# OpenGVLab/MM-Interleaved

Hardware: NVIDIA H100
Metric: interleaved_steps_per_sec (higher is better)
Workload: dtype bf16

## Files before the change

### mm-interleaved_b200/csrc/attn_fwd_sm100.cu

```cuda
#include "attn_common.cuh"

namespace mmfs {

constexpr int kBM = 128, kBN = 64;
constexpr int kAttnThreads = 288;
constexpr int kConsumers = 256;

template <int HD> constexpr int attn_ctas_per_sm() { return HD == 64 ? 2 : 1; }

template <typename T, int HD>
__global__ void __launch_bounds__(kAttnThreads, attn_ctas_per_sm<HD>())
attn_fwd_kernel(const __grid_constant__ CUtensorMap map_q, const __grid_constant__ CUtensorMap map_k,
                const __grid_constant__ CUtensorMap map_v, const AttnParams p, unsigned *__restrict__ sched, int n_work) {
    constexpr int NBOX = HD / 64;
    constexpr uint32_t QBOX_BYTES = kBM * 128, KBOX_BYTES = kBN * 128;
    constexpr uint32_t Q_BYTES = NBOX * QBOX_BYTES, KV_BYTES = NBOX * KBOX_BYTES;
    extern __shared__ __align__(1024) uint8_t smem_raw[];
    if ((s_addr(smem_raw) & 1023u) != 0u) { asm volatile("trap;"); }
    uint8_t *sQ = smem_raw;
    uint8_t *sK = sQ + Q_BYTES;
    uint8_t *sV = sK + 2 * KV_BYTES;
    uint64_t *bars = reinterpret_cast<uint64_t *>(sV + 2 * KV_BYTES);
    uint64_t *q_full = bars + 0, *q_empty = bars + 1, *k_full = bars + 2 , *k_empty = bars + 4 ,
             *v_full = bars + 6 , *v_empty = bars + 8 , *item_full = bars + 10 , *item_empty = bars + 12 ;
    int *s_item = reinterpret_cast<int *>(bars + 14);

    const int warp = threadIdx.x >> 5, lane = threadIdx.x & 31;
    const int n_q = (p.Tq + kBM - 1) / kBM;
    auto decode = [&](int w, int &h, int &b, int &q0, int &n_tiles) {
        b = w / (n_q * p.H);
        const int r = w - b * (n_q * p.H);
        const int mi = r / p.H;
        h = r - mi * p.H;
        q0 = (p.causal ? n_q - 1 - mi : mi) * kBM;
        int kv_end = p.Tkv;
        if (p.causal) kv_end = min(p.Tkv, p.past + min(q0 + kBM, p.Tq));
        n_tiles = (kv_end + kBN - 1) / kBN;
    };

    if (threadIdx.x == 0) {
        bar_init(q_full, 1);
        bar_init(q_empty, kConsumers);
        for (int i = 0; i < 2; ++i) {
            bar_init(k_full + i, 1); bar_init(v_full + i, 1); bar_init(k_empty + i, kConsumers); bar_init(v_empty + i, kConsumers);
            bar_init(item_full + i, 1); bar_init(item_empty + i, kConsumers);
        }
        asm volatile("fence.mbarrier_init.release.cluster;" ::: "memory");
    }
    __syncthreads();

    if (warp == 8) {
        if (lane == 0) {
            int w = blockIdx.x;
            int g = 0;
            for (int qn = 0;; ++qn) {
                const int slot = qn & 1;
                if (qn >= 2) bar_wait(item_empty + slot, ((qn >> 1) - 1) & 1);
                s_item[slot] = w < n_work ? w : -1;
                bar_arrive(item_full + slot);
                if (w >= n_work) break;
                const int w_next = sched ? (int)gridDim.x + (int)atomicAdd(sched, 1u) : n_work;
                int h, b, q0, n_tiles;
                decode(w, h, b, q0, n_tiles);
                if (qn > 0) bar_wait(q_empty, (qn - 1) & 1);
                bar_expect_tx(q_full, Q_BYTES);
#pragma unroll
                for (int bx = 0; bx < NBOX; ++bx) tma_load_4d(sQ + bx * QBOX_BYTES, &map_q, q_full, bx * 64, h, q0, b);
                for (int j = 0; j < n_tiles; ++j, ++g) {
                    const int s = g & 1;
                    const uint32_t ph = (g >> 1) & 1;
                    bar_wait(k_empty + s, ph ^ 1);
                    bar_expect_tx(k_full + s, KV_BYTES);
#pragma unroll
                    for (int bx = 0; bx < NBOX; ++bx)
                        tma_load_4d(sK + s * KV_BYTES + bx * KBOX_BYTES, &map_k, k_full + s, bx * 64, h, j * kBN, b);
                    bar_wait(v_empty + s, ph ^ 1);
                    bar_expect_tx(v_full + s, KV_BYTES);
#pragma unroll
                    for (int bx = 0; bx < NBOX; ++bx)
                        tma_load_4d(sV + s * KV_BYTES + bx * KBOX_BYTES, &map_v, v_full + s, bx * 64, h, j * kBN, b);
                }
                w = w_next;
            }
        }
        return;
    }

    const int wg = warp >> 2;
    const int quad = lane >> 2, tq = lane & 3;
    const int row_in_tile = wg * 64 + (warp & 3) * 16 + quad;
    const uint32_t q_base = s_addr(sQ) + wg * 64 * 128;
    int g = 0;
    for (int qn = 0;; ++qn) {
        const int slot = qn & 1;
        bar_wait(item_full + slot, (qn >> 1) & 1);
        const int w = s_item[slot];
        bar_arrive(item_empty + slot);
        if (w < 0) break;
        int h, b, q0, n_tiles;
        decode(w, h, b, q0, n_tiles);
        const int r0 = q0 + row_in_tile;
        float m_run[2] = {-INFINITY, -INFINITY}, l_run[2] = {0.f, 0.f};
        float o[HD / 2];
#pragma unroll
        for (int i = 0; i < HD / 2; ++i) o[i] = 0.f;
        bar_wait(q_full, qn & 1);
        if (n_tiles == 0) bar_arrive(q_empty);

        for (int j = 0; j < n_tiles; ++j, ++g) {
            const int s = g & 1;
            const int k0 = j * kBN;
            float sc[kBN / 2];
            bar_wait(k_full + s, (g >> 1) & 1);
            wgmma_fence();
#pragma unroll
            for (int kk = 0; kk < HD / 16; ++kk)
                Wgmma<T>::ss_n64(sc, smem_desc(q_base + (kk >> 2) * QBOX_BYTES + (kk & 3) * 32, 16, 1024),
                                 smem_desc(s_addr(sK) + s * KV_BYTES + (kk >> 2) * KBOX_BYTES + (kk & 3) * 32, 16, 1024), kk > 0);
            wgmma_commit();
            wgmma_wait<0>();
            reg_fence(sc);
            bar_arrive(k_empty + s);
            if (j + 1 == n_tiles) bar_arrive(q_empty);

            const bool need_mask = (k0 + kBN > p.Tkv) || (p.key_mask != nullptr) ||
                                   (p.causal && k0 + kBN - 1 > p.past + q0 + wg * 64);
            if (need_mask) {
#pragma unroll
                for (int jj = 0; jj < kBN / 8; ++jj)
#pragma unroll
                    for (int c = 0; c < 2; ++c) {
                        const int key = k0 + jj * 8 + 2 * tq + c;
                        bool vis = key < p.Tkv;
                        if (vis && p.key_mask != nullptr) vis = p.key_mask[(long)b * p.Tkv + key] != 0;
#pragma unroll
                        for (int i = 0; i < 2; ++i) {
                            const bool ok = vis && (!p.causal || key <= p.past + r0 + 8 * i);
                            if (!ok) sc[jj * 4 + 2 * i + c] = -INFINITY;
                        }
                    }
            }
            float alpha[2], neg_m[2];
#pragma unroll
            for (int i = 0; i < 2; ++i) {
                float mx = -INFINITY;
#pragma unroll
                for (int jj = 0; jj < kBN / 8; ++jj) mx = fmaxf(mx, fmaxf(sc[jj * 4 + 2 * i], sc[jj * 4 + 2 * i + 1]));
                mx = fmaxf(mx, __shfl_xor_sync(0xffffffffu, mx, 1));
                mx = fmaxf(mx, __shfl_xor_sync(0xffffffffu, mx, 2));
                const float m_new = fmaxf(m_run[i], mx);
                alpha[i] = (m_new == -INFINITY) ? 1.f : fast_exp2((m_run[i] - m_new) * p.scale_log2e);
                m_run[i] = m_new;
                neg_m[i] = (m_new == -INFINITY) ? 0.f : -m_new * p.scale_log2e;
            }
            uint32_t pa[kBN / 16][4];
            float ls[2] = {0.f, 0.f};
#pragma unroll
            for (int jj = 0; jj < kBN / 8; ++jj)
#pragma unroll
                for (int i = 0; i < 2; ++i) {
                    const float e0 = fast_exp2(fmaf(sc[jj * 4 + 2 * i], p.scale_log2e, neg_m[i]));
                    const float e1 = fast_exp2(fmaf(sc[jj * 4 + 2 * i + 1], p.scale_log2e, neg_m[i]));
                    ls[i] += e0 + e1;
                    pa[jj >> 1][(jj & 1) * 2 + i] = pack2<T>(e0, e1);
                }
#pragma unroll
            for (int i = 0; i < 2; ++i) l_run[i] = l_run[i] * alpha[i] + ls[i];
#pragma unroll
            for (int jj = 0; jj < HD / 8; ++jj) {
                o[jj * 4 + 0] *= alpha[0]; o[jj * 4 + 1] *= alpha[0];
                o[jj * 4 + 2] *= alpha[1]; o[jj * 4 + 3] *= alpha[1];
            }

            bar_wait(v_full + s, (g >> 1) & 1);
            reg_fence(o);
            wgmma_fence();
#pragma unroll
            for (int kk = 0; kk < kBN / 16; ++kk) {
                const uint64_t dv = smem_desc(s_addr(sV) + s * KV_BYTES + kk * 16 * 128, KBOX_BYTES, 1024);
                if constexpr (HD == 64) Wgmma<T>::rs_n64(o, pa[kk], dv, 1);
                else Wgmma<T>::rs_n128(o, pa[kk], dv, 1);
            }
            wgmma_commit();
            wgmma_wait<0>();
            reg_fence(o);
            bar_arrive(v_empty + s);
        }

        T *out = static_cast<T *>(p.out) + (long)b * p.o_bs + (long)h * HD;
#pragma unroll
        for (int i = 0; i < 2; ++i) {
            float l = l_run[i];
            l += __shfl_xor_sync(0xffffffffu, l, 1);
            l += __shfl_xor_sync(0xffffffffu, l, 2);
            const float inv = (l > 0.f) ? 1.f / l : 0.f;
            const int q = r0 + 8 * i;
            if (q < p.Tq) {
                T *op = out + (long)q * p.o_ts + 2 * tq;
#pragma unroll
                for (int jj = 0; jj < HD / 8; ++jj)
                    *reinterpret_cast<uint32_t *>(op + jj * 8) = pack2<T>(o[jj * 4 + 2 * i] * inv, o[jj * 4 + 2 * i + 1] * inv);
            }
        }
    }
}

struct MapKey {
    const void *ptr; int dtype, B, T, H, hd, box_rows; long bs, ts;
    bool operator==(const MapKey &o) const {
        return ptr == o.ptr && dtype == o.dtype && B == o.B && T == o.T && H == o.H && hd == o.hd && box_rows == o.box_rows &&
               bs == o.bs && ts == o.ts;
    }
};
constexpr int kMapCache = 32;
static thread_local MapKey g_map_keys[kMapCache];
static thread_local CUtensorMap g_map_vals[kMapCache];
static thread_local int g_map_n = 0, g_map_next = 0;

static int make_map_uncached(CUtensorMap *map, const void *ptr, int dtype, int B, int T, int H, int hd, long bs, long ts, int box_rows);

static int make_map(CUtensorMap *map, const void *ptr, int dtype, int B, int T, int H, int hd, long bs, long ts, int box_rows) {
    const MapKey key{ptr, dtype, B, T, H, hd, box_rows, bs, ts};
    for (int i = 0; i < g_map_n; ++i)
        if (g_map_keys[i] == key) { *map = g_map_vals[i]; return MMFS_OK; }
    const int rc = make_map_uncached(map, ptr, dtype, B, T, H, hd, bs, ts, box_rows);
    if (rc != MMFS_OK) return rc;
    g_map_keys[g_map_next] = key;
    g_map_vals[g_map_next] = *map;
    g_map_next = (g_map_next + 1) % kMapCache;
    if (g_map_n < kMapCache) ++g_map_n;
    return MMFS_OK;
}

static int make_map_uncached(CUtensorMap *map, const void *ptr, int dtype, int B, int T, int H, int hd, long bs, long ts, int box_rows) {
    EncodeTiledFn fn = tensor_map_encoder();
    if (!fn) { set_error("attn: cuTensorMapEncodeTiled is not available from this driver"); return MMFS_ECUDA; }
    const cuuint64_t dims[4] = {(cuuint64_t)hd, (cuuint64_t)H, (cuuint64_t)T, (cuuint64_t)B};
    const cuuint64_t strides[3] = {(cuuint64_t)hd * 2, (cuuint64_t)ts * 2, (cuuint64_t)bs * 2};
    const cuuint32_t box[4] = {64, 1, (cuuint32_t)box_rows, 1};
    const cuuint32_t estr[4] = {1, 1, 1, 1};
    CUresult r = fn(map, dtype == MMFS_BF16 ? CU_TENSOR_MAP_DATA_TYPE_BFLOAT16 : CU_TENSOR_MAP_DATA_TYPE_FLOAT16, 4,
                    const_cast<void *>(ptr), dims, strides, box, estr, CU_TENSOR_MAP_INTERLEAVE_NONE,
                    CU_TENSOR_MAP_SWIZZLE_128B, CU_TENSOR_MAP_L2_PROMOTION_L2_128B, CU_TENSOR_MAP_FLOAT_OOB_FILL_NONE);
    if (r != CUDA_SUCCESS) { set_error("attn: cuTensorMapEncodeTiled failed (%d)", (int)r); return MMFS_ECUDA; }
    return MMFS_OK;
}

template <typename T, int HD>
static int launch_attn(const CUtensorMap &mq, const CUtensorMap &mk, const CUtensorMap &mv, const AttnParams &p,
                       unsigned *work_counter, cudaStream_t st) {
    const int n_q = (p.Tq + kBM - 1) / kBM;
    const long n_work = (long)n_q * p.H * p.B;
    if (n_work >= (1L << 30)) { set_error("attn_forward: %ld work items", n_work); return MMFS_EUNSUPPORTED; }
    constexpr size_t smem = (size_t)(HD / 64) * (kBM * 128 + 4 * kBN * 128) + 14 * 8 + 2 * sizeof(int);
    constexpr auto kern = attn_fwd_kernel<T, HD>;
    const int rc = ensure_dynamic_smem<kern>(smem);
    if (rc != MMFS_OK) return rc;
    const int resident = attn_ctas_per_sm<HD>() * num_sms();
    const bool persistent = n_work > resident;
    if (persistent) MMFS_CUDA(cudaMemsetAsync(work_counter, 0, sizeof(unsigned), st));
    const int grid = persistent ? resident : (int)n_work;
    kern<<<grid, kAttnThreads, smem, st>>>(mq, mk, mv, p, persistent ? work_counter : nullptr, (int)n_work);
    MMFS_CUDA(cudaGetLastError());
    return MMFS_OK;
}

}

using namespace mmfs;

extern "C" int mmfs_attn_forward(const void *q, const void *k, const void *v, void *out, const uint8_t *key_mask,
                                 int B, int H, int Tq, int Tkv, int hd,
                                 long q_bs, long q_ts, long k_bs, long k_ts, long v_bs, long v_ts, long o_bs, long o_ts,
                                 float scale, int causal, int past, int dtype, unsigned *work_counter, void *stream) {
    MMFS_CHECK_ARG(B >= 0 && H > 0 && Tq >= 0 && Tkv > 0, "attn_forward: bad shape");
    if (B == 0 || Tq == 0) return MMFS_OK;
    MMFS_CHECK_ARG(q && k && v && out && work_counter, "attn_forward: null pointer argument");
    MMFS_CHECK_ARG((uintptr_t)work_counter % 4 == 0, "attn_forward: work_counter must be 4-byte aligned");
    if (!(hd == 64 || hd == 128) || !(dtype == MMFS_BF16 || dtype == MMFS_F16)) {
        set_error("attn_forward: tensor-core path needs hd in {64,128} and bf16/f16 (got hd=%d dtype=%d)", hd, dtype);
        return MMFS_EUNSUPPORTED;
    }
    if (((uintptr_t)q | (uintptr_t)k | (uintptr_t)v | (uintptr_t)out) % 16 != 0 ||
        (q_bs | q_ts | k_bs | k_ts | v_bs | v_ts | o_bs | o_ts) % 8 != 0 || B > 65535 || H > 65535) {
        set_error("attn_forward: pointers / strides must be 16-byte aligned; B, H <= 65535");
        return MMFS_EUNSUPPORTED;
    }
    CUtensorMap mq, mk, mv;
    int rc;
    if ((rc = make_map(&mq, q, dtype, B, Tq, H, hd, q_bs, q_ts, kBM)) != MMFS_OK) return rc;
    if ((rc = make_map(&mk, k, dtype, B, Tkv, H, hd, k_bs, k_ts, kBN)) != MMFS_OK) return rc;
    if ((rc = make_map(&mv, v, dtype, B, Tkv, H, hd, v_bs, v_ts, kBN)) != MMFS_OK) return rc;
    AttnParams p;
    p.out = out; p.key_mask = key_mask; p.B = B; p.H = H; p.Tq = Tq; p.Tkv = Tkv; p.causal = causal; p.past = past;
    p.o_bs = o_bs; p.o_ts = o_ts; p.scale_log2e = scale * 1.4426950408889634f;
    cudaStream_t st = (cudaStream_t)stream;
    return dispatch_dtype<kF16Types>(dtype, "attn_forward", [&](auto tag) {
        using T = typename decltype(tag)::type;
        return hd == 64 ? launch_attn<T, 64>(mq, mk, mv, p, work_counter, st) : launch_attn<T, 128>(mq, mk, mv, p, work_counter, st);
    });
}
```

### mm-interleaved_b200/csrc/tc_common.cuh

```cuda
#pragma once
#include <cuda.h>

#include "common.cuh"

namespace mmfs {

__device__ __forceinline__ void tma_load_4d(void *dst, const CUtensorMap *map, uint64_t *bar, int c0, int c1, int c2, int c3) {
    asm volatile(
        "cp.async.bulk.tensor.4d.shared::cluster.global.mbarrier::complete_tx::bytes [%0], [%1, {%3, %4, %5, %6}], [%2];" ::
        "r"(s_addr(dst)), "l"(map), "r"(s_addr(bar)), "r"(c0), "r"(c1), "r"(c2), "r"(c3) : "memory");
}
__device__ __forceinline__ void fence_async_smem() { asm volatile("fence.proxy.async.shared::cta;" ::: "memory"); }

__device__ __forceinline__ void wgmma_fence() { asm volatile("wgmma.fence.sync.aligned;" ::: "memory"); }
__device__ __forceinline__ void wgmma_commit() { asm volatile("wgmma.commit_group.sync.aligned;" ::: "memory"); }
template <int N> __device__ __forceinline__ void wgmma_wait() { asm volatile("wgmma.wait_group.sync.aligned %0;" ::"n"(N) : "memory"); }
template <int N> __device__ __forceinline__ void reg_fence(float (&d)[N]) {
#pragma unroll
    for (int i = 0; i < N; ++i) asm volatile("" : "+f"(d[i])::"memory");
}

__device__ __forceinline__ uint64_t smem_desc(uint32_t saddr, uint32_t lbo_bytes, uint32_t sbo_bytes) {
    return (uint64_t)((saddr >> 4) & 0x3fffu) | ((uint64_t)((lbo_bytes >> 4) & 0x3fffu) << 16) |
           ((uint64_t)((sbo_bytes >> 4) & 0x3fffu) << 32) | (1ull << 62);
}

template <typename T> struct Wgmma;
#define MMFS_WGMMA_OPS(TY) \
     \
    __device__ __forceinline__ static void ss_n64(float (&d)[32], uint64_t da, uint64_t db, int acc) { \
        asm volatile( \
            "{\n\t.reg .pred p;\n\tsetp.ne.b32 p, %34, 0;\n\t" \
            "wgmma.mma_async.sync.aligned.m64n64k16.f32." TY "." TY " {%0,%1,%2,%3,%4,%5,%6,%7,%8,%9,%10,%11,%12,%13,%14,%15,%16,%17,%18,%19,%20,%21,%22,%23,%24,%25,%26,%27,%28,%29,%30,%31}, %32, %33, p, 1, 1, 0, 0;\n\t}" \
            : "+f"(d[0]), "+f"(d[1]), "+f"(d[2]), "+f"(d[3]), "+f"(d[4]), "+f"(d[5]), "+f"(d[6]), "+f"(d[7]), "+f"(d[8]), "+f"(d[9]), "+f"(d[10]), "+f"(d[11]), "+f"(d[12]), "+f"(d[13]), "+f"(d[14]), "+f"(d[15]), "+f"(d[16]), "+f"(d[17]), "+f"(d[18]), "+f"(d[19]), "+f"(d[20]), "+f"(d[21]), "+f"(d[22]), "+f"(d[23]), "+f"(d[24]), "+f"(d[25]), "+f"(d[26]), "+f"(d[27]), "+f"(d[28]), "+f"(d[29]), "+f"(d[30]), "+f"(d[31]) \
            : "l"(da), "l"(db), "r"(acc)); \
    } \
     \
    __device__ __forceinline__ static void ss_n128(float (&d)[64], uint64_t da, uint64_t db, int acc) { \
        asm volatile( \
            "{\n\t.reg .pred p;\n\tsetp.ne.b32 p, %66, 0;\n\t" \
            "wgmma.mma_async.sync.aligned.m64n128k16.f32." TY "." TY " {%0,%1,%2,%3,%4,%5,%6,%7,%8,%9,%10,%11,%12,%13,%14,%15,%16,%17,%18,%19,%20,%21,%22,%23,%24,%25,%26,%27,%28,%29,%30,%31,%32,%33,%34,%35,%36,%37,%38,%39,%40,%41,%42,%43,%44,%45,%46,%47,%48,%49,%50,%51,%52,%53,%54,%55,%56,%57,%58,%59,%60,%61,%62,%63}, %64, %65, p, 1, 1, 0, 0;\n\t}" \
            : "+f"(d[0]), "+f"(d[1]), "+f"(d[2]), "+f"(d[3]), "+f"(d[4]), "+f"(d[5]), "+f"(d[6]), "+f"(d[7]), "+f"(d[8]), "+f"(d[9]), "+f"(d[10]), "+f"(d[11]), "+f"(d[12]), "+f"(d[13]), "+f"(d[14]), "+f"(d[15]), "+f"(d[16]), "+f"(d[17]), "+f"(d[18]), "+f"(d[19]), "+f"(d[20]), "+f"(d[21]), "+f"(d[22]), "+f"(d[23]), "+f"(d[24]), "+f"(d[25]), "+f"(d[26]), "+f"(d[27]), "+f"(d[28]), "+f"(d[29]), "+f"(d[30]), "+f"(d[31]), "+f"(d[32]), "+f"(d[33]), "+f"(d[34]), "+f"(d[35]), "+f"(d[36]), "+f"(d[37]), "+f"(d[38]), "+f"(d[39]), "+f"(d[40]), "+f"(d[41]), "+f"(d[42]), "+f"(d[43]), "+f"(d[44]), "+f"(d[45]), "+f"(d[46]), "+f"(d[47]), "+f"(d[48]), "+f"(d[49]), "+f"(d[50]), "+f"(d[51]), "+f"(d[52]), "+f"(d[53]), "+f"(d[54]), "+f"(d[55]), "+f"(d[56]), "+f"(d[57]), "+f"(d[58]), "+f"(d[59]), "+f"(d[60]), "+f"(d[61]), "+f"(d[62]), "+f"(d[63]) \
            : "l"(da), "l"(db), "r"(acc)); \
    } \
     \
    __device__ __forceinline__ static void ss_n160(float (&d)[80], uint64_t da, uint64_t db, int acc) { \
        asm volatile( \
            "{\n\t.reg .pred p;\n\tsetp.ne.b32 p, %82, 0;\n\t" \
            "wgmma.mma_async.sync.aligned.m64n160k16.f32." TY "." TY " {%0,%1,%2,%3,%4,%5,%6,%7,%8,%9,%10,%11,%12,%13,%14,%15,%16,%17,%18,%19,%20,%21,%22,%23,%24,%25,%26,%27,%28,%29,%30,%31,%32,%33,%34,%35,%36,%37,%38,%39,%40,%41,%42,%43,%44,%45,%46,%47,%48,%49,%50,%51,%52,%53,%54,%55,%56,%57,%58,%59,%60,%61,%62,%63,%64,%65,%66,%67,%68,%69,%70,%71,%72,%73,%74,%75,%76,%77,%78,%79}, %80, %81, p, 1, 1, 0, 0;\n\t}" \
            : "+f"(d[0]), "+f"(d[1]), "+f"(d[2]), "+f"(d[3]), "+f"(d[4]), "+f"(d[5]), "+f"(d[6]), "+f"(d[7]), "+f"(d[8]), "+f"(d[9]), "+f"(d[10]), "+f"(d[11]), "+f"(d[12]), "+f"(d[13]), "+f"(d[14]), "+f"(d[15]), "+f"(d[16]), "+f"(d[17]), "+f"(d[18]), "+f"(d[19]), "+f"(d[20]), "+f"(d[21]), "+f"(d[22]), "+f"(d[23]), "+f"(d[24]), "+f"(d[25]), "+f"(d[26]), "+f"(d[27]), "+f"(d[28]), "+f"(d[29]), "+f"(d[30]), "+f"(d[31]), "+f"(d[32]), "+f"(d[33]), "+f"(d[34]), "+f"(d[35]), "+f"(d[36]), "+f"(d[37]), "+f"(d[38]), "+f"(d[39]), "+f"(d[40]), "+f"(d[41]), "+f"(d[42]), "+f"(d[43]), "+f"(d[44]), "+f"(d[45]), "+f"(d[46]), "+f"(d[47]), "+f"(d[48]), "+f"(d[49]), "+f"(d[50]), "+f"(d[51]), "+f"(d[52]), "+f"(d[53]), "+f"(d[54]), "+f"(d[55]), "+f"(d[56]), "+f"(d[57]), "+f"(d[58]), "+f"(d[59]), "+f"(d[60]), "+f"(d[61]), "+f"(d[62]), "+f"(d[63]), "+f"(d[64]), "+f"(d[65]), "+f"(d[66]), "+f"(d[67]), "+f"(d[68]), "+f"(d[69]), "+f"(d[70]), "+f"(d[71]), "+f"(d[72]), "+f"(d[73]), "+f"(d[74]), "+f"(d[75]), "+f"(d[76]), "+f"(d[77]), "+f"(d[78]), "+f"(d[79]) \
            : "l"(da), "l"(db), "r"(acc)); \
    } \
     \
    __device__ __forceinline__ static void rs_n64(float (&d)[32], const uint32_t (&a)[4], uint64_t db, int acc) { \
        asm volatile( \
            "{\n\t.reg .pred p;\n\tsetp.ne.b32 p, %37, 0;\n\t" \
            "wgmma.mma_async.sync.aligned.m64n64k16.f32." TY "." TY " {%0,%1,%2,%3,%4,%5,%6,%7,%8,%9,%10,%11,%12,%13,%14,%15,%16,%17,%18,%19,%20,%21,%22,%23,%24,%25,%26,%27,%28,%29,%30,%31}, {%32,%33,%34,%35}, %36, p, 1, 1, 1;\n\t}" \
            : "+f"(d[0]), "+f"(d[1]), "+f"(d[2]), "+f"(d[3]), "+f"(d[4]), "+f"(d[5]), "+f"(d[6]), "+f"(d[7]), "+f"(d[8]), "+f"(d[9]), "+f"(d[10]), "+f"(d[11]), "+f"(d[12]), "+f"(d[13]), "+f"(d[14]), "+f"(d[15]), "+f"(d[16]), "+f"(d[17]), "+f"(d[18]), "+f"(d[19]), "+f"(d[20]), "+f"(d[21]), "+f"(d[22]), "+f"(d[23]), "+f"(d[24]), "+f"(d[25]), "+f"(d[26]), "+f"(d[27]), "+f"(d[28]), "+f"(d[29]), "+f"(d[30]), "+f"(d[31]) \
            : "r"(a[0]), "r"(a[1]), "r"(a[2]), "r"(a[3]), "l"(db), "r"(acc)); \
    } \
     \
    __device__ __forceinline__ static void rs_n128(float (&d)[64], const uint32_t (&a)[4], uint64_t db, int acc) { \
        asm volatile( \
            "{\n\t.reg .pred p;\n\tsetp.ne.b32 p, %69, 0;\n\t" \
            "wgmma.mma_async.sync.aligned.m64n128k16.f32." TY "." TY " {%0,%1,%2,%3,%4,%5,%6,%7,%8,%9,%10,%11,%12,%13,%14,%15,%16,%17,%18,%19,%20,%21,%22,%23,%24,%25,%26,%27,%28,%29,%30,%31,%32,%33,%34,%35,%36,%37,%38,%39,%40,%41,%42,%43,%44,%45,%46,%47,%48,%49,%50,%51,%52,%53,%54,%55,%56,%57,%58,%59,%60,%61,%62,%63}, {%64,%65,%66,%67}, %68, p, 1, 1, 1;\n\t}" \
            : "+f"(d[0]), "+f"(d[1]), "+f"(d[2]), "+f"(d[3]), "+f"(d[4]), "+f"(d[5]), "+f"(d[6]), "+f"(d[7]), "+f"(d[8]), "+f"(d[9]), "+f"(d[10]), "+f"(d[11]), "+f"(d[12]), "+f"(d[13]), "+f"(d[14]), "+f"(d[15]), "+f"(d[16]), "+f"(d[17]), "+f"(d[18]), "+f"(d[19]), "+f"(d[20]), "+f"(d[21]), "+f"(d[22]), "+f"(d[23]), "+f"(d[24]), "+f"(d[25]), "+f"(d[26]), "+f"(d[27]), "+f"(d[28]), "+f"(d[29]), "+f"(d[30]), "+f"(d[31]), "+f"(d[32]), "+f"(d[33]), "+f"(d[34]), "+f"(d[35]), "+f"(d[36]), "+f"(d[37]), "+f"(d[38]), "+f"(d[39]), "+f"(d[40]), "+f"(d[41]), "+f"(d[42]), "+f"(d[43]), "+f"(d[44]), "+f"(d[45]), "+f"(d[46]), "+f"(d[47]), "+f"(d[48]), "+f"(d[49]), "+f"(d[50]), "+f"(d[51]), "+f"(d[52]), "+f"(d[53]), "+f"(d[54]), "+f"(d[55]), "+f"(d[56]), "+f"(d[57]), "+f"(d[58]), "+f"(d[59]), "+f"(d[60]), "+f"(d[61]), "+f"(d[62]), "+f"(d[63]) \
            : "r"(a[0]), "r"(a[1]), "r"(a[2]), "r"(a[3]), "l"(db), "r"(acc)); \
    }
template <> struct Wgmma<__nv_bfloat16> { MMFS_WGMMA_OPS("bf16") };
template <> struct Wgmma<__half> { MMFS_WGMMA_OPS("f16") };
#undef MMFS_WGMMA_OPS


__device__ __forceinline__ void tma_load_2d(void *dst, const CUtensorMap *map, uint64_t *bar, int c0, int c1) {
    asm volatile(
        "cp.async.bulk.tensor.2d.shared::cluster.global.mbarrier::complete_tx::bytes [%0], [%1, {%3, %4}], [%2];" ::
        "r"(s_addr(dst)), "l"(map), "r"(s_addr(bar)), "r"(c0), "r"(c1) : "memory");
}

typedef CUresult (*EncodeTiledFn)(CUtensorMap *, CUtensorMapDataType, cuuint32_t, void *, const cuuint64_t *, const cuuint64_t *,
                                  const cuuint32_t *, const cuuint32_t *, CUtensorMapInterleave, CUtensorMapSwizzle,
                                  CUtensorMapL2promotion, CUtensorMapFloatOOBfill);

inline EncodeTiledFn tensor_map_encoder() {
    static EncodeTiledFn fn = nullptr;
    if (!fn) {
        void *ptr = nullptr;
        cudaDriverEntryPointQueryResult qres;
        if (cudaGetDriverEntryPoint("cuTensorMapEncodeTiled", &ptr, cudaEnableDefault, &qres) == cudaSuccess &&
            qres == cudaDriverEntryPointSuccess)
            fn = (EncodeTiledFn)ptr;
    }
    return fn;
}

}
```

Baseline: 1.920.

## Pipeline QK^T and PV wgmma with 128-key tiles and register reallocation

Raises the key/value tile from 64 to 128 keys and splits each tile's softmax into two 64-key halves. The consumer loop is software-pipelined so the next tile's QK^T wgmma overlaps the previous tile's PV wgmma and softmax math. A fourth producer warpgroup is added so setmaxnreg can move registers from the producers to the consumers. In exchange, head dim 64 drops from two CTAs per SM to one, shared memory per CTA doubles for K/V, and the fence and wait ordering becomes more complex and more error-prone.

```diff
diff --git a/mm-interleaved_b200/csrc/attn_fwd_sm100.cu b/mm-interleaved_b200/csrc/attn_fwd_sm100.cu
--- a/mm-interleaved_b200/csrc/attn_fwd_sm100.cu
+++ b/mm-interleaved_b200/csrc/attn_fwd_sm100.cu
@@ -2,18 +2,28 @@
 
 namespace mmfs {
 
-constexpr int kBM = 128, kBN = 64;
-constexpr int kAttnThreads = 288;
+constexpr int kBM = 128;
+constexpr int kAttnThreads = 384;
 constexpr int kConsumers = 256;
 
-template <int HD> constexpr int attn_ctas_per_sm() { return HD == 64 ? 2 : 1; }
+template <int HD> struct AttnTile {
+    static constexpr int BN = 128;
+    static constexpr int CTAS = 1;
+    static constexpr int CONSUMER_REGS = 232, PRODUCER_REGS = 40;
+};
+
+template <int HD> constexpr size_t attn_smem_bytes() {
+    return (size_t)(HD / 64) * (kBM * 128 + 4 * AttnTile<HD>::BN * 128) + 14 * 8 + 2 * sizeof(int);
+}
 
 template <typename T, int HD>
-__global__ void __launch_bounds__(kAttnThreads, attn_ctas_per_sm<HD>())
+__global__ void __launch_bounds__(kAttnThreads, AttnTile<HD>::CTAS)
 attn_fwd_kernel(const __grid_constant__ CUtensorMap map_q, const __grid_constant__ CUtensorMap map_k,
                 const __grid_constant__ CUtensorMap map_v, const AttnParams p, unsigned *__restrict__ sched, int n_work) {
+    using Tile = AttnTile<HD>;
+    constexpr int BN = Tile::BN;
     constexpr int NBOX = HD / 64;
-    constexpr uint32_t QBOX_BYTES = kBM * 128, KBOX_BYTES = kBN * 128;
+    constexpr uint32_t QBOX_BYTES = kBM * 128, KBOX_BYTES = BN * 128;
     constexpr uint32_t Q_BYTES = NBOX * QBOX_BYTES, KV_BYTES = NBOX * KBOX_BYTES;
     extern __shared__ __align__(1024) uint8_t smem_raw[];
     if ((s_addr(smem_raw) & 1023u) != 0u) { asm volatile("trap;"); }
@@ -28,14 +38,14 @@
     const int warp = threadIdx.x >> 5, lane = threadIdx.x & 31;
     const int n_q = (p.Tq + kBM - 1) / kBM;
     auto decode = [&](int w, int &h, int &b, int &q0, int &n_tiles) {
-        b = w / (n_q * p.H);
+        b = (unsigned)w / (unsigned)(n_q * p.H);
         const int r = w - b * (n_q * p.H);
-        const int mi = r / p.H;
+        const int mi = (unsigned)r / (unsigned)p.H;
         h = r - mi * p.H;
         q0 = (p.causal ? n_q - 1 - mi : mi) * kBM;
         int kv_end = p.Tkv;
         if (p.causal) kv_end = min(p.Tkv, p.past + min(q0 + kBM, p.Tq));
-        n_tiles = (kv_end + kBN - 1) / kBN;
+        n_tiles = (kv_end + BN - 1) / BN;
     };
 
     if (threadIdx.x == 0) {
@@ -49,8 +59,9 @@
     }
     __syncthreads();
 
-    if (warp == 8) {
-        if (lane == 0) {
+    if (warp >= 8) {
+        setmaxnreg_dec<Tile::PRODUCER_REGS>();
+        if (warp == 8 && lane == 0) {
             int w = blockIdx.x;
             int g = 0;
             for (int qn = 0;; ++qn) {
@@ -71,14 +82,14 @@
                     const uint32_t ph = (g >> 1) & 1;
                     bar_wait(k_empty + s, ph ^ 1);
                     bar_expect_tx(k_full + s, KV_BYTES);
-#pragma unroll
+#pragma unroll 1
                     for (int bx = 0; bx < NBOX; ++bx)
-                        tma_load_4d(sK + s * KV_BYTES + bx * KBOX_BYTES, &map_k, k_full + s, bx * 64, h, j * kBN, b);
+                        tma_load_4d(sK + s * KV_BYTES + bx * KBOX_BYTES, &map_k, k_full + s, bx * 64, h, j * BN, b);
                     bar_wait(v_empty + s, ph ^ 1);
                     bar_expect_tx(v_full + s, KV_BYTES);
-#pragma unroll
+#pragma unroll 1
                     for (int bx = 0; bx < NBOX; ++bx)
-                        tma_load_4d(sV + s * KV_BYTES + bx * KBOX_BYTES, &map_v, v_full + s, bx * 64, h, j * kBN, b);
+                        tma_load_4d(sV + s * KV_BYTES + bx * KBOX_BYTES, &map_v, v_full + s, bx * 64, h, j * BN, b);
                 }
                 w = w_next;
             }
@@ -86,10 +97,37 @@
         return;
     }
 
+    setmaxnreg_inc<Tile::CONSUMER_REGS>();
     const int wg = warp >> 2;
     const int quad = lane >> 2, tq = lane & 3;
     const int row_in_tile = wg * 64 + (warp & 3) * 16 + quad;
     const uint32_t q_base = s_addr(sQ) + wg * 64 * 128;
+
+    static_assert(BN == 128, "two 64-key softmax steps per K / V tile");
+
+    auto issue_s = [&](float (&sc)[BN / 2], int gt) {
+        const int s = gt & 1;
+        bar_wait(k_full + s, (gt >> 1) & 1);
+#pragma unroll
+        for (int kk = 0; kk < HD / 16; ++kk) {
+            const uint64_t da = smem_desc(q_base + (kk >> 2) * QBOX_BYTES + (kk & 3) * 32, 16, 1024);
+            const uint64_t db = smem_desc(s_addr(sK) + s * KV_BYTES + (kk >> 2) * KBOX_BYTES + (kk & 3) * 32, 16, 1024);
+            Wgmma<T>::ss_n128(sc, da, db, kk > 0);
+        }
+        wgmma_commit();
+    };
+    auto issue_pv = [&](float (&o)[HD / 2], uint32_t (&pa)[BN / 16][4], int gt, int hf) {
+        const int s = gt & 1;
+        bar_wait(v_full + s, (gt >> 1) & 1);
+#pragma unroll
+        for (int kk = hf * 4; kk < hf * 4 + 4; ++kk) {
+            const uint64_t dv = smem_desc(s_addr(sV) + s * KV_BYTES + kk * 16 * 128, KBOX_BYTES, 1024);
+            if constexpr (HD == 64) Wgmma<T>::rs_n64(o, pa[kk], dv, 1);
+            else Wgmma<T>::rs_n128(o, pa[kk], dv, 1);
+        }
+        wgmma_commit();
+    };
+
     int g = 0;
     for (int qn = 0;; ++qn) {
         const int slot = qn & 1;
@@ -104,30 +142,17 @@
         float o[HD / 2];
 #pragma unroll
         for (int i = 0; i < HD / 2; ++i) o[i] = 0.f;
+        float sc[BN / 2];
+        uint32_t pa[BN / 16][4];
         bar_wait(q_full, qn & 1);
         if (n_tiles == 0) bar_arrive(q_empty);
 
-        for (int j = 0; j < n_tiles; ++j, ++g) {
-            const int s = g & 1;
-            const int k0 = j * kBN;
-            float sc[kBN / 2];
-            bar_wait(k_full + s, (g >> 1) & 1);
-            wgmma_fence();
-#pragma unroll
-            for (int kk = 0; kk < HD / 16; ++kk)
-                Wgmma<T>::ss_n64(sc, smem_desc(q_base + (kk >> 2) * QBOX_BYTES + (kk & 3) * 32, 16, 1024),
-                                 smem_desc(s_addr(sK) + s * KV_BYTES + (kk >> 2) * KBOX_BYTES + (kk & 3) * 32, 16, 1024), kk > 0);
-            wgmma_commit();
-            wgmma_wait<0>();
-            reg_fence(sc);
-            bar_arrive(k_empty + s);
-            if (j + 1 == n_tiles) bar_arrive(q_empty);
-
-            const bool need_mask = (k0 + kBN > p.Tkv) || (p.key_mask != nullptr) ||
-                                   (p.causal && k0 + kBN - 1 > p.past + q0 + wg * 64);
+        auto softmax = [&](int k0, int hf, float (&alpha)[2]) {
+            const bool need_mask = (k0 + 64 > p.Tkv) || (p.key_mask != nullptr) ||
+                                   (p.causal && k0 + 63 > p.past + q0 + wg * 64);
             if (need_mask) {
 #pragma unroll
-                for (int jj = 0; jj < kBN / 8; ++jj)
+                for (int jj = 0; jj < 8; ++jj)
 #pragma unroll
                     for (int c = 0; c < 2; ++c) {
                         const int key = k0 + jj * 8 + 2 * tq + c;
@@ -136,16 +161,16 @@
 #pragma unroll
                         for (int i = 0; i < 2; ++i) {
                             const bool ok = vis && (!p.causal || key <= p.past + r0 + 8 * i);
-                            if (!ok) sc[jj * 4 + 2 * i + c] = -INFINITY;
+                            if (!ok) sc[(hf * 8 + jj) * 4 + 2 * i + c] = -INFINITY;
                         }
                     }
             }
-            float alpha[2], neg_m[2];
+            float neg_m[2];
 #pragma unroll
             for (int i = 0; i < 2; ++i) {
                 float mx = -INFINITY;
 #pragma unroll
-                for (int jj = 0; jj < kBN / 8; ++jj) mx = fmaxf(mx, fmaxf(sc[jj * 4 + 2 * i], sc[jj * 4 + 2 * i + 1]));
+                for (int jj = hf * 8; jj < hf * 8 + 8; ++jj) mx = fmaxf(mx, fmaxf(sc[jj * 4 + 2 * i], sc[jj * 4 + 2 * i + 1]));
                 mx = fmaxf(mx, __shfl_xor_sync(0xffffffffu, mx, 1));
                 mx = fmaxf(mx, __shfl_xor_sync(0xffffffffu, mx, 2));
                 const float m_new = fmaxf(m_run[i], mx);
@@ -153,39 +178,93 @@
                 m_run[i] = m_new;
                 neg_m[i] = (m_new == -INFINITY) ? 0.f : -m_new * p.scale_log2e;
             }
-            uint32_t pa[kBN / 16][4];
             float ls[2] = {0.f, 0.f};
 #pragma unroll
-            for (int jj = 0; jj < kBN / 8; ++jj)
+            for (int jj = hf * 8; jj < hf * 8 + 8; ++jj)
 #pragma unroll
                 for (int i = 0; i < 2; ++i) {
-                    const float e0 = fast_exp2(fmaf(sc[jj * 4 + 2 * i], p.scale_log2e, neg_m[i]));
-                    const float e1 = fast_exp2(fmaf(sc[jj * 4 + 2 * i + 1], p.scale_log2e, neg_m[i]));
+                    float &e0 = sc[jj * 4 + 2 * i], &e1 = sc[jj * 4 + 2 * i + 1];
+                    e0 = fast_exp2(fmaf(e0, p.scale_log2e, neg_m[i]));
+                    e1 = fast_exp2(fmaf(e1, p.scale_log2e, neg_m[i]));
                     ls[i] += e0 + e1;
-                    pa[jj >> 1][(jj & 1) * 2 + i] = pack2<T>(e0, e1);
                 }
 #pragma unroll
             for (int i = 0; i < 2; ++i) l_run[i] = l_run[i] * alpha[i] + ls[i];
+        };
+        auto pack_p = [&](int hf) {
+#pragma unroll
+            for (int jj = hf * 8; jj < hf * 8 + 8; ++jj)
+#pragma unroll
+                for (int i = 0; i < 2; ++i) pa[jj >> 1][(jj & 1) * 2 + i] = pack2<T>(sc[jj * 4 + 2 * i], sc[jj * 4 + 2 * i + 1]);
+        };
+        auto rescale_o = [&](const float (&alpha)[2]) {
 #pragma unroll
             for (int jj = 0; jj < HD / 8; ++jj) {
                 o[jj * 4 + 0] *= alpha[0]; o[jj * 4 + 1] *= alpha[0];
                 o[jj * 4 + 2] *= alpha[1]; o[jj * 4 + 3] *= alpha[1];
             }
-
-            bar_wait(v_full + s, (g >> 1) & 1);
-            reg_fence(o);
-            wgmma_fence();
-#pragma unroll
-            for (int kk = 0; kk < kBN / 16; ++kk) {
-                const uint64_t dv = smem_desc(s_addr(sV) + s * KV_BYTES + kk * 16 * 128, KBOX_BYTES, 1024);
-                if constexpr (HD == 64) Wgmma<T>::rs_n64(o, pa[kk], dv, 1);
-                else Wgmma<T>::rs_n128(o, pa[kk], dv, 1);
-            }
-            wgmma_commit();
-            wgmma_wait<0>();
-            reg_fence(o);
-            bar_arrive(v_empty + s);
-        }
+        };
+
+        float alpha_b[2];
+        if (n_tiles > 0) {
+            float alpha_a[2];
+            wgmma_fence();
+            issue_s(sc, g);
+            wgmma_wait<0>();
+            reg_fence(sc);
+            bar_arrive(k_empty + (g & 1));
+            if (n_tiles == 1) bar_arrive(q_empty);
+            softmax(0, 0, alpha_a);
+            softmax(64, 1, alpha_b);
+            pack_p(0);
+            pack_p(1);
+        }
+        for (int j = 1; j < n_tiles; ++j) {
+            const int gj = g + j, k0 = j * BN;
+            float alpha_a[2];
+            reg_fence(o);
+            wgmma_fence();
+            issue_s(sc, gj);
+            issue_pv(o, pa, gj - 1, 0);
+            wgmma_wait<1>();
+            reg_fence(sc);
+            bar_arrive(k_empty + (gj & 1));
+            if (j + 1 == n_tiles) bar_arrive(q_empty);
+            softmax(k0, 0, alpha_a);
+            wgmma_wait<0>();
+            reg_fence(o);
+            reg_fence(pa);
+            rescale_o(alpha_b);
+            reg_fence(o);
+            wgmma_fence();
+            issue_pv(o, pa, gj - 1, 1);
+            pack_p(0);
+            softmax(k0 + 64, 1, alpha_b);
+            wgmma_wait<0>();
+            reg_fence(o);
+            reg_fence(pa);
+            bar_arrive(v_empty + ((gj - 1) & 1));
+            rescale_o(alpha_a);
+            pack_p(1);
+        }
+        if (n_tiles > 0) {
+            const int gl = g + n_tiles - 1;
+            reg_fence(o);
+            wgmma_fence();
+            issue_pv(o, pa, gl, 0);
+            wgmma_wait<0>();
+            reg_fence(o);
+            reg_fence(pa);
+            rescale_o(alpha_b);
+            reg_fence(o);
+            wgmma_fence();
+            issue_pv(o, pa, gl, 1);
+            wgmma_wait<0>();
+            reg_fence(o);
+            reg_fence(pa);
+            bar_arrive(v_empty + (gl & 1));
+        }
+        g += n_tiles;
 
         T *out = static_cast<T *>(p.out) + (long)b * p.o_bs + (long)h * HD;
 #pragma unroll
@@ -252,11 +331,11 @@
     const int n_q = (p.Tq + kBM - 1) / kBM;
     const long n_work = (long)n_q * p.H * p.B;
     if (n_work >= (1L << 30)) { set_error("attn_forward: %ld work items", n_work); return MMFS_EUNSUPPORTED; }
-    constexpr size_t smem = (size_t)(HD / 64) * (kBM * 128 + 4 * kBN * 128) + 14 * 8 + 2 * sizeof(int);
+    constexpr size_t smem = attn_smem_bytes<HD>();
     constexpr auto kern = attn_fwd_kernel<T, HD>;
     const int rc = ensure_dynamic_smem<kern>(smem);
     if (rc != MMFS_OK) return rc;
-    const int resident = attn_ctas_per_sm<HD>() * num_sms();
+    const int resident = AttnTile<HD>::CTAS * num_sms();
     const bool persistent = n_work > resident;
     if (persistent) MMFS_CUDA(cudaMemsetAsync(work_counter, 0, sizeof(unsigned), st));
     const int grid = persistent ? resident : (int)n_work;
@@ -287,10 +366,11 @@
         return MMFS_EUNSUPPORTED;
     }
     CUtensorMap mq, mk, mv;
+    const int bn = hd == 64 ? AttnTile<64>::BN : AttnTile<128>::BN;
     int rc;
     if ((rc = make_map(&mq, q, dtype, B, Tq, H, hd, q_bs, q_ts, kBM)) != MMFS_OK) return rc;
-    if ((rc = make_map(&mk, k, dtype, B, Tkv, H, hd, k_bs, k_ts, kBN)) != MMFS_OK) return rc;
-    if ((rc = make_map(&mv, v, dtype, B, Tkv, H, hd, v_bs, v_ts, kBN)) != MMFS_OK) return rc;
+    if ((rc = make_map(&mk, k, dtype, B, Tkv, H, hd, k_bs, k_ts, bn)) != MMFS_OK) return rc;
+    if ((rc = make_map(&mv, v, dtype, B, Tkv, H, hd, v_bs, v_ts, bn)) != MMFS_OK) return rc;
     AttnParams p;
     p.out = out; p.key_mask = key_mask; p.B = B; p.H = H; p.Tq = Tq; p.Tkv = Tkv; p.causal = causal; p.past = past;
     p.o_bs = o_bs; p.o_ts = o_ts; p.scale_log2e = scale * 1.4426950408889634f;
diff --git a/mm-interleaved_b200/csrc/tc_common.cuh b/mm-interleaved_b200/csrc/tc_common.cuh
--- a/mm-interleaved_b200/csrc/tc_common.cuh
+++ b/mm-interleaved_b200/csrc/tc_common.cuh
@@ -19,6 +19,15 @@
 #pragma unroll
     for (int i = 0; i < N; ++i) asm volatile("" : "+f"(d[i])::"memory");
 }
+template <int M, int N> __device__ __forceinline__ void reg_fence(uint32_t (&a)[M][N]) {
+#pragma unroll
+    for (int i = 0; i < M; ++i)
+#pragma unroll
+        for (int j = 0; j < N; ++j) asm volatile("" : "+r"(a[i][j])::"memory");
+}
+
+template <int R> __device__ __forceinline__ void setmaxnreg_inc() { asm volatile("setmaxnreg.inc.sync.aligned.u32 %0;" ::"n"(R)); }
+template <int R> __device__ __forceinline__ void setmaxnreg_dec() { asm volatile("setmaxnreg.dec.sync.aligned.u32 %0;" ::"n"(R)); }
 
 __device__ __forceinline__ uint64_t smem_desc(uint32_t saddr, uint32_t lbo_bytes, uint32_t sbo_bytes) {
     return (uint64_t)((saddr >> 4) & 0x3fffu) | ((uint64_t)((lbo_bytes >> 4) & 0x3fffu) << 16) |
```

Measured after the change: 1.923 (median of 6 runs). Within noise of the previous version (+0.1%).
